# zju3dv/OnePose_Plus_Plus

Hardware: AMD Instinct MI355X
Metric: query images/sec (2D-3D match fwd) at 512x512 img x 5k pts (higher is better)
Workload: dtype f32 (operands as exact bf16 triples, f32 accumulate)

## Files before the change

onepose_plus_plus_amd/csrc/gemm_mfma.hip:

```cpp
#include <stdlib.h>

#include <mutex>
#include <type_traits>

#include <vector>

#include "opp_internal.h"

typedef float f32x16 __attribute__((ext_vector_type(16)));
typedef _Float16 f16x8 __attribute__((ext_vector_type(8)));
typedef __bf16 bf16x8 __attribute__((ext_vector_type(8)));
typedef __bf16 bf16x2 __attribute__((ext_vector_type(2)));
typedef float f32x2 __attribute__((ext_vector_type(2)));

namespace {

constexpr int lds_stride(int prec) { return prec == OPP_PREC_BF16X3 ? 52 : 36; }

__device__ __forceinline__ void opp_split4_b3(const float4 v, uint2& hi, uint2& mid, uint2& lo) {
  auto lvl = [](float a, float b, float& ra, float& rb) -> unsigned {
    const f32x2 t = {a, b};
    const unsigned p = __builtin_bit_cast(unsigned, __builtin_convertvector(t, bf16x2));
    ra = a - __uint_as_float(p << 16);
    rb = b - __uint_as_float(p & 0xffff0000u);
// ... 5 lines not shown
  const unsigned l01 = lvl(s0, s1, u0, u1), l23 = lvl(s2, s3, u2, u3);
  hi = make_uint2(h01, h23);
  mid = make_uint2(m01, m23);
  lo = make_uint2(l01, l23);
}
__device__ __forceinline__ void opp_store_split4(void* base, size_t row_bytes_off, int col, const float4 v) {
  uint2 hi, mid, lo;
  opp_split4_b3(v, hi, mid, lo);
  char* p = static_cast<char*>(base) + row_bytes_off + (col >> 3) * 48 + (col & 7) * 2;
  *reinterpret_cast<uint2*>(p) = hi;
  *reinterpret_cast<uint2*>(p + 16) = mid;
  *reinterpret_cast<uint2*>(p + 32) = lo;
}

template <int BM, int BN, int WAVES_M, int WAVES_N, bool CONV, int ABL, int DEPTH, int PREC, bool ASP>
__device__ __forceinline__ void opp_gemm_body(const OppGemm& g) {
  constexpr bool H2 = PREC == OPP_PREC_FP16X2;
  constexpr bool H3 = PREC == OPP_PREC_BF16X3;
  constexpr int kLdsStride = lds_stride(PREC);
  constexpr int NT = WAVES_M * WAVES_N * 64;
  constexpr int TM = BM / WAVES_M / 32;
  constexpr int NT32 = BN / 32;
  constexpr int TN = (NT32 + WAVES_N - 1) / WAVES_N;
  constexpr bool kRagged = (NT32 % WAVES_N) != 0;
  static_assert(!ASP || (CONV && PREC == OPP_PREC_BF16X3 && (ABL == 0 || ABL >= 200)), "pre-split activations: bf16x3 convolutions only");
  constexpr int kAblMask = ABL >= 200 ? ABL - 200 : 0;
  constexpr bool kNoGload = ABL == 91 || (kAblMask & 1), kNoLdsSt = ABL == 92 || (kAblMask & 2), kNoBar = ABL == 93 || (kAblMask & 4),
                 kNoFrag = ABL == 94 || (kAblMask & 8);
  constexpr int A_LD = ASP ? (BM * 12 + NT - 1) / NT : BM * 8 / NT;
  constexpr bool kAFrac = ASP && (BM * 12) % NT != 0;
  constexpr int kBRowsLoad = (H3 && BN == 224) ? 208 : BN;
  constexpr int B_LD = H3 ? (kBRowsLoad * 12 + NT - 1) / NT : BN * 8 / NT;
  constexpr bool kBFrac = H3 && (kBRowsLoad * 12) % NT != 0;
  constexpr bool kRing = H3 && kRagged;
  static_assert(BM % (WAVES_M * 32) == 0 && BN % 32 == 0, "tile shape");
  static_assert((BM * 8) % NT == 0 && (H3 ? (BN * 12) % NT == 0 || BN == 192 || BN == 224 : (BN * 8) % NT == 0), "load split");
  static_assert(!ASP || !((H3 && ((BN + 31) / 32 % WAVES_N) != 0)), "pre-split activations are not built for the ring tile");

  unsigned long long ts0 = 0, ts1 = 0, ts2 = 0;
  if (ABL == 9 || ABL > 90) ts0 = __builtin_readcyclecounter();
  extern __shared__ __attribute__((aligned(16))) float smem[];
  float* As = smem;
  float* Bs = smem + 2 * BM * kLdsStride;

  const int tid = threadIdx.x;
  const int lane = tid & 63;
  const int wave = tid >> 6;
  const int wm = __builtin_amdgcn_readfirstlane(kRing ? wave % WAVES_M : wave / WAVES_N);
  const int wn = __builtin_amdgcn_readfirstlane(kRing ? wave / WAVES_M : wave % WAVES_N);
  bool tile_ok[TN];
#pragma unroll
  for (int j = 0; j < TN; ++j) tile_ok[j] = kRagged ? (wn * TN + j < NT32) : true;
  const int half = lane >> 5;
  const int l31 = lane & 31;

  const int tiles_n = (g.n_store + BN - 1) / BN;
  int tile_lin = blockIdx.x;
  if (g.xcd_swizzle & 1) {
    const int nb = gridDim.x, q = nb >> 3, r = nb & 7;
    const int xcd = blockIdx.x & 7, idx = blockIdx.x >> 3;
    tile_lin = (xcd < r ? xcd * (q + 1) : r * (q + 1) + (xcd - r) * q) + idx;
  }
  const int tile_m = tile_lin / tiles_n;
  const int tile_n = tile_lin - tile_m * tiles_n;
  const int m0 = tile_m * BM;
  const int n0 = tile_n * BN;

  const int kq = tid & 7;
  const int lrow = tid >> 3;

  constexpr unsigned kOob = 0x80000000u;

  unsigned a_base0[A_LD], a_base1[A_LD], a_mask[A_LD];
  int a_lds[ASP ? A_LD : 1];
#pragma unroll
  for (int i = 0; i < A_LD; ++i) {
    const int au = tid + i * NT;
    const int arow = ASP ? au / 12 : lrow + i * (NT / 8);
    const int apiece = ASP ? au - arow * 12 : 0;
    if constexpr (ASP) a_lds[i] = arow * kLdsStride + apiece * 4;
    const int r = m0 + arow;
    if (CONV) {
      const int ox = r % g.Wout;
      const int t = r / g.Wout;
      const int oy = t % g.Hout;
      const int b = t / g.Hout;
      const int iy0 = oy * g.stride - g.pad;
      const int ix0 = ox * g.stride - g.pad;
      if constexpr (ASP) a_base0[i] = (unsigned)(((b * g.Hin + iy0) * g.Win + ix0) * g.Cin) * 6u + (unsigned)apiece * 16u;
      else a_base0[i] = (unsigned)(((b * g.Hin + iy0) * g.Win + ix0) * g.Cin + kq * 4) * 4u;
      a_base1[i] = 0;
      unsigned m = 0;
#pragma unroll
      for (int ky = 0; ky < 3; ++ky)
#pragma unroll
        for (int kx = 0; kx < 3; ++kx) {
          const bool ok = ky < g.ksize && kx < g.ksize && (unsigned)(iy0 + ky) < (unsigned)g.Hin &&
                          (unsigned)(ix0 + kx) < (unsigned)g.Win;
          m |= (ok ? 1u : 0u) << (ky * g.ksize + kx);
        }
      a_mask[i] = (r < g.M && (!kAFrac || au < BM * 12)) ? ~m : 0xffffffffu;
    } else {
      a_base0[i] = r < g.M ? (unsigned)(r * g.lda0 + kq * 4) * 4u : kOob;
      a_base1[i] = r < g.M ? (unsigned)(r * g.lda1 + kq * 4) * 4u : kOob;
      a_mask[i] = 0;
    }
  }
  constexpr bool kRingB = H3 && (NT32 % WAVES_N) != 0;
  unsigned b_base[kRingB ? 1 : B_LD];
  int b_lds[kRingB ? 1 : B_LD];
  auto ring_b = [&](int i, unsigned& base, int& lds) {
    int t = tid;
    asm volatile("" : "+v"(t));
    const int u = t + i * NT;
    const int row = u / 12, c = u - row * 12;
    const int n = n0 + row;
    base = (n < g.N && u < kBRowsLoad * 12) ? (unsigned)(n * g.ldw + c * 4) * 4u : kOob;
    lds = row * kLdsStride + c * 4;
  };
#pragma unroll
  for (int i = 0; i < (kRingB ? 0 : B_LD); ++i) {
    if (H3) {
      const int u = tid + i * NT;
      const int row = u / 12, c = u - row * 12;
      const int n = n0 + row;
      if constexpr (kBFrac) b_base[i] = (n < g.N && u < kBRowsLoad * 12) ? (unsigned)(n * g.ldw + c * 4) * 4u : kOob;
      else b_base[i] = n < g.N ? (unsigned)(n * g.ldw + c * 4) * 4u : kOob;
      b_lds[i] = row * kLdsStride + c * 4;
    } else {
      const int n = n0 + lrow + i * (NT / 8);
      b_base[i] = n < g.N ? (unsigned)(n * g.ldw + kq * 4) * 4u : kOob;
      b_lds[i] = (lrow + i * (NT / 8)) * kLdsStride + kq * 4;
    }
  }

  typedef unsigned int u32x4 __attribute__((ext_vector_type(4)));
  auto bload = [](const __amdgpu_buffer_rsrc_t r, unsigned off) -> float4 {
    const u32x4 v = __builtin_amdgcn_raw_buffer_load_b128(r, (int)off, 0, 0);
    return make_float4(__uint_as_float(v.x), __uint_as_float(v.y), __uint_as_float(v.z), __uint_as_float(v.w));
  };

  const int k_first = g.k_splits > 1 ? (int)blockIdx.y * g.k_chunks_per_split : 0;
  const int nk = g.k_splits > 1 ? max(0, min(g.k_chunks_per_split, g.K / 32 - k_first)) : g.K / 32;
  const int taps = CONV ? g.ksize * g.ksize : 1;
  const int ngrp = CONV ? g.Cin / 32 : nk;
  int cur_i = 0;
  int cur_grp = 0;
  int cur_tap = 0, cur_ky = 0, cur_kx = 0;
  int cur_k0 = k_first * 32;
  unsigned cur_past = nk > 0 ? 0u : kOob;
  unsigned eff_delta = 0, eff_sh = 31;
  int tail_i = -1;
  const int kq_lane = tid & 7;
  auto tail_lane = [&](int t, unsigned& delta, unsigned& sh) {
    const int tp = t * 8 + kq_lane;
    const int ty = tp / g.ksize, tx = tp - ty * g.ksize;
    delta = (unsigned)((ty * g.Win + tx) * g.Cin + g.tail_grp * 32 - kq_lane * 4) * 4u;
    sh = (unsigned)(31 - tp);
  };
  auto step_cursor = [&]() {
    if (CONV) {
// ... 67 lines not shown
  };
  auto load_global = [&](float4 (&a_reg)[A_LD], float4 (&b_reg)[B_LD]) {
#pragma unroll
    for (int i = 0; i < A_LD + B_LD; ++i) load_item(i, a_reg, b_reg);
  };

  auto split_h2 = [](const float4 v, uint2& hi, uint2& lo) {
    const unsigned h01 = __builtin_bit_cast(unsigned, __builtin_amdgcn_cvt_pkrtz(v.x, v.y));
    const unsigned h23 = __builtin_bit_cast(unsigned, __builtin_amdgcn_cvt_pkrtz(v.z, v.w));
    unsigned l01, l23;
    asm("v_fma_mixlo_f16 %0, %1, -1.0, %2 op_sel:[0,0,0] op_sel_hi:[1,0,0]" : "=v"(l01) : "v"(h01), "v"(v.x));
    asm("v_fma_mixhi_f16 %0, %1, -1.0, %2 op_sel:[1,0,0] op_sel_hi:[1,0,0]" : "+v"(l01) : "v"(h01), "v"(v.y));
    asm("v_fma_mixlo_f16 %0, %1, -1.0, %2 op_sel:[0,0,0] op_sel_hi:[1,0,0]" : "=v"(l23) : "v"(h23), "v"(v.z));
    asm("v_fma_mixhi_f16 %0, %1, -1.0, %2 op_sel:[1,0,0] op_sel_hi:[1,0,0]" : "+v"(l23) : "v"(h23), "v"(v.w));
    hi = make_uint2(h01, h23);
    lo = make_uint2(l01, l23);
  };
  auto split_b3 = [](const float4 v, uint2& hi, uint2& mid, uint2& lo) { opp_split4_b3(v, hi, mid, lo); };
  auto store_item = [&](int i, int buf, const float4 (&a_reg)[A_LD], const float4 (&b_reg)[B_LD]) {
    if (i < A_LD) {
      if constexpr (ASP) {
        if (!kAFrac || tid + i * NT < BM * 12) *reinterpret_cast<float4*>(As + buf * BM * kLdsStride + a_lds[i]) = a_reg[i];
        return;
      }
      float* row = As + buf * BM * kLdsStride + (lrow + i * (NT / 8)) * kLdsStride;
      if (H3) {
        uint2 hi, mid, lo;
        if (ABL == 95) {
          hi = make_uint2(__float_as_uint(a_reg[i].x), __float_as_uint(a_reg[i].y));
          mid = make_uint2(__float_as_uint(a_reg[i].z), __float_as_uint(a_reg[i].w));
          lo = hi;
        } else
        split_b3(a_reg[i], hi, mid, lo);
        float* dst = row + (kq >> 1) * 12 + (kq & 1) * 2;
        *reinterpret_cast<uint2*>(dst) = hi;
        *reinterpret_cast<uint2*>(dst + 4) = mid;
        *reinterpret_cast<uint2*>(dst + 8) = lo;
      } else if (H2) {
        uint2 hi, lo;
        split_h2(a_reg[i], hi, lo);
        float* dst = row + (kq >> 1) * 8 + (kq & 1) * 2;
        *reinterpret_cast<uint2*>(dst) = hi;
        *reinterpret_cast<uint2*>(dst + 4) = lo;
      } else {
        *reinterpret_cast<float4*>(row + kq * 4) = a_reg[i];
      }
    } else {
      if constexpr (kRingB) {
        unsigned base;
        int lds;
        ring_b(i - A_LD, base, lds);
        if (tid + (i - A_LD) * NT < kBRowsLoad * 12) *reinterpret_cast<float4*>(Bs + buf * BN * kLdsStride + lds) = b_reg[i - A_LD];
      } else if constexpr (kBFrac) {
        if (tid + (i - A_LD) * NT < kBRowsLoad * 12) *reinterpret_cast<float4*>(Bs + buf * BN * kLdsStride + b_lds[i - A_LD]) = b_reg[i - A_LD];
      } else {
        *reinterpret_cast<float4*>(Bs + buf * BN * kLdsStride + b_lds[i - A_LD]) = b_reg[i - A_LD];
      }
    }
  };
  auto store_lds = [&](int buf, const float4 (&a_reg)[A_LD], const float4 (&b_reg)[B_LD]) {
#pragma unroll
    for (int i = 0; i < A_LD + B_LD; ++i) store_item(i, buf, a_reg, b_reg);
  };

  f32x16 acc[TM][TN];
#pragma unroll
  for (int i = 0; i < TM; ++i)
// ... 13 lines not shown
    for (int i = 0; i < TM; ++i) af[i] = *reinterpret_cast<const float4*>(as + i * 32 * kLdsStride);
#pragma unroll
    for (int j = 0; j < TN; ++j)
      if (tile_ok[j]) bf[j] = *reinterpret_cast<const float4*>(bs + j * 32 * kLdsStride);
  };
  auto mfma_quarter = [&](const float4 (&af)[TM], const float4 (&bf)[TN], auto&& between) {
    int n = 0;
#pragma unroll
    for (int e = 0; e < 4; ++e) {
#pragma unroll
      for (int i = 0; i < TM; ++i) {
#pragma unroll
        for (int j = 0; j < TN; ++j) {
          if (tile_ok[j]) {
            const float av = e == 0 ? af[i].x : e == 1 ? af[i].y : e == 2 ? af[i].z : af[i].w;
            const float bv = e == 0 ? bf[j].x : e == 1 ? bf[j].y : e == 2 ? bf[j].z : bf[j].w;
            acc[i][j] = __builtin_amdgcn_mfma_f32_32x32x2f32(av, bv, acc[i][j], 0, 0, 0);
          }
          between(n);
          ++n;
        }
      }
    }
  };
  auto nothing = [](int) {};
  constexpr int kSlots = TM * TN * 4;
  constexpr int kItems = A_LD + B_LD;
  constexpr int kStride = kSlots / kItems > 0 ? kSlots / kItems : 1;

  float4 ga[DEPTH][A_LD], gb[DEPTH][B_LD];
  float4 fa[(H3 && !kRing) ? 6 : 4][TM], fb[(H3 && !kRing) ? 6 : 4][TN];
  float4 da[A_LD], db[B_LD];

  if constexpr (kRing) {
    load_global(ga[0], gb[0]);
  } else {
#pragma unroll
    for (int d = 0; d < DEPTH; ++d) {
      if (d) advance();
      load_global(ga[d], gb[d]);
    }
  }
  if constexpr (kBRowsLoad < BN) {
    for (int u = tid; u < 2 * (BN - kBRowsLoad) * kLdsStride; u += NT) {
      const int b = u / ((BN - kBRowsLoad) * kLdsStride), o = u - b * ((BN - kBRowsLoad) * kLdsStride);
      Bs[b * BN * kLdsStride + kBRowsLoad * kLdsStride + o] = 0.f;
    }
  }
  store_lds(0, ga[0], gb[0]);
  if constexpr (kRing) {
    __builtin_amdgcn_sched_barrier(0);
    advance();
    load_global(ga[1], gb[0]);
  }
  __syncthreads();
  read_frags(0, 0, fa[0], fb[0]);
  if constexpr (kRing) {
    read_frags(0, 1, fa[2], fb[2]);
    read_frags(0, 2, fa[3], fb[3]);
  } else {
    if (H2 || H3) read_frags(0, 1, fa[1], fb[1]);
    if constexpr (H3) read_frags(0, 2, fa[(H3 && !kRing) ? 2 : 0], fb[(H3 && !kRing) ? 2 : 0]);
  }

  auto chunk = [&](auto set, int lb) {
    constexpr int P = decltype(set)::value;
    constexpr int PN = (P + 1) % DEPTH;
    constexpr int A2 = ABL == 5 ? 1 : (ABL >= 6 ? 0 : ABL);
    const int B0 = A2 >= 2 ? 0 : lb;
    const int B1 = A2 >= 2 ? 0 : lb ^ 1;
    if (ABL < 1 || ABL >= 5) advance();
    if (A2 < 3) read_frags(B0, 1, fa[1], fb[1]);
    __builtin_amdgcn_sched_barrier(0);
    mfma_quarter(fa[0], fb[0], [&](int n) {
      if ((ABL < 1 || ABL >= 5) && n % kStride == 0 && n / kStride < kItems) {
        if (ABL == 5) load_item(n / kStride, da, db);
        else load_item(n / kStride, ga[P], gb[P]);
        __builtin_amdgcn_sched_barrier(0);
      }
    });
    if (ABL < 1 || ABL >= 6) {
#pragma unroll
      for (int i = kSlots / kStride; i < kItems; ++i) load_item(i, ga[P], gb[P]);
    }
    __builtin_amdgcn_sched_barrier(0);
    if (A2 < 3) read_frags(B0, 2, fa[0], fb[0]);
    __builtin_amdgcn_sched_barrier(0);
    mfma_quarter(fa[1], fb[1], nothing);
    __builtin_amdgcn_sched_barrier(0);
    if (A2 < 3) read_frags(B0, 3, fa[1], fb[1]);
// ... 207 lines not shown
    read_frags_n(B0, 5, fa[3], fb[3], tnw_c);
    __builtin_amdgcn_sched_barrier(0);
    mfma_ring(0, 2, 5, 2 * TM * TNW, tnw_c, pre);
    __builtin_amdgcn_sched_barrier(0);
    read_frags_n(B0, 4, fa[2], fb[2], tnw_c);
    __builtin_amdgcn_sched_barrier(0);
    mfma_ring(0, 5, 6, 5 * TM * TNW, tnw_c, pre);
#pragma unroll
    for (int i = kSlotsR0 / kStrideR0; i < A_LD; ++i) load_item(i, ga[P], gb[0]);
    __builtin_amdgcn_sched_barrier(0);
    mfma_ring(1, 0, 3, 0, tnw_c, [&](int n) {
      if (n % kStrideR1 == 0 && n / kStrideR1 < kItems) {
        store_item(n / kStrideR1, B1, ga[PN], gb[0]);
        __builtin_amdgcn_sched_barrier(0);
      }
    });
#pragma unroll
    for (int i = kSlotsR1 / kStrideR1; i < kItems; ++i) store_item(i, B1, ga[PN], gb[0]);
    __builtin_amdgcn_sched_barrier(0);
    __syncthreads();
    read_frags_n(B1, 0, fa[0], fb[0], tnw_c);
    read_frags_n(B1, 2, fa[3], fb[3], tnw_c);
    __builtin_amdgcn_sched_barrier(0);
    mfma_ring(1, 3, 5, 0, tnw_c, pre_b);
    __builtin_amdgcn_sched_barrier(0);
    read_frags_n(B1, 1, fa[2], fb[2], tnw_c);
    __builtin_amdgcn_sched_barrier(0);
    mfma_ring(1, 5, 6, 2 * TM * TNW, tnw_c, pre_b);
#pragma unroll
    for (int i = kSlotsR1 / kStrideRB; i < B_LD; ++i) load_item(A_LD + i, ga[P], gb[0]);
    __builtin_amdgcn_sched_barrier(0);
  };

  if (ABL == 9 || ABL > 90) ts1 = __builtin_readcyclecounter();
  if (NT == 512 && (g.xcd_swizzle & 2) && __builtin_amdgcn_readfirstlane(tid) >= 256) __builtin_amdgcn_s_setprio(1);
  if constexpr (kRing) {
    constexpr int kFull = TN, kShort = NT32 - (WAVES_N - 1) * TN;
    static_assert(DEPTH == 2 && kShort >= 1 && kShort <= TN, "ring tile");
    if (wn != WAVES_N - 1) {
      for (int c = 0; c < nk; c += 2) {
        chunk_ring(std::integral_constant<int, 0>{}, c & 1, std::integral_constant<int, kFull>{});
        chunk_ring(std::integral_constant<int, 1>{}, (c + 1) & 1, std::integral_constant<int, kFull>{});
      }
    } else {
      for (int c = 0; c < nk; c += 2) {
        chunk_ring(std::integral_constant<int, 0>{}, c & 1, std::integral_constant<int, kShort>{});
        chunk_ring(std::integral_constant<int, 1>{}, (c + 1) & 1, std::integral_constant<int, kShort>{});
      }
    }
  }
  for (int c = 0; c < (kRing ? 0 : nk); c += DEPTH) {
    if constexpr (kRing) {
    } else if constexpr (H3) {
      chunk_h3(std::integral_constant<int, 0>{}, c & 1);
      if (DEPTH > 1) chunk_h3(std::integral_constant<int, 1 % DEPTH>{}, (c + 1) & 1);
      if (DEPTH > 2) chunk_h3(std::integral_constant<int, 2 % DEPTH>{}, (c + 2) & 1);
      if (DEPTH > 3) chunk_h3(std::integral_constant<int, 3 % DEPTH>{}, (c + 3) & 1);
    } else if constexpr (H2) {
      chunk_h2(std::integral_constant<int, 0>{}, c & 1);
      if (DEPTH > 1) chunk_h2(std::integral_constant<int, 1 % DEPTH>{}, (c + 1) & 1);
      if (DEPTH > 2) chunk_h2(std::integral_constant<int, 2 % DEPTH>{}, (c + 2) & 1);
      if (DEPTH > 3) chunk_h2(std::integral_constant<int, 3 % DEPTH>{}, (c + 3) & 1);
    } else {
      chunk(std::integral_constant<int, 0>{}, c & 1);
      if (DEPTH > 1) chunk(std::integral_constant<int, 1 % DEPTH>{}, (c + 1) & 1);
      if (DEPTH > 2) chunk(std::integral_constant<int, 2 % DEPTH>{}, (c + 2) & 1);
      if (DEPTH > 3) chunk(std::integral_constant<int, 3 % DEPTH>{}, (c + 3) & 1);
    }
  }
  if (ABL == 9 || ABL > 90) ts2 = __builtin_readcyclecounter();
  if (ABL == 5) {
#pragma unroll
    for (int i = 0; i < A_LD; ++i) asm volatile("" ::"v"(da[i].x), "v"(da[i].w));
#pragma unroll
    for (int i = 0; i < B_LD; ++i) asm volatile("" ::"v"(db[i].x), "v"(db[i].w));
  }

  constexpr int kJPmax = TN < 4 ? TN : 4;
  constexpr int kOperandFloats = 2 * (BM + BN) * kLdsStride;
  constexpr int JP = (BM * (WAVES_N * kJPmax * 32 + 4) <= kOperandFloats) ? kJPmax
                     : (BM * (WAVES_N * 2 * 32 + 4) <= kOperandFloats && kJPmax >= 2) ? 2 : 1;
  constexpr int NPASS = (TN + JP - 1) / JP;
  constexpr int WP = WAVES_N * JP * 32;
  constexpr int CS = WP + 4;
  static_assert((size_t)BM * CS * 4 <= (size_t)2 * (BM + BN) * kLdsStride * 4, "C tile must fit the operand LDS");
  float* Cs = smem;
  const bool scale_on = (g.out_mul != 1.f) || (g.out_div != 1.f);
  const bool vec_ok = g.vec_epilogue != 0;
  const float h2_inv = (H2 && g.h2_inv != nullptr) ? *g.h2_inv : 1.f;
  if (H2 || scale_on) {
#pragma unroll
    for (int i = 0; i < TM; ++i)
#pragma unroll
      for (int j = 0; j < TN; ++j)
#pragma unroll
        for (int r = 0; r < 16; ++r) {
          const float cv0 = H2 ? acc[i][j][r] * h2_inv : acc[i][j][r];
          acc[i][j][r] = scale_on ? (cv0 * g.out_mul) / g.out_div : cv0;
        }
  }
  if (g.col_mask != nullptr) {
#pragma unroll
    for (int j = 0; j < TN; ++j) {
      const int col = n0 + wn * TN * 32 + j * 32 + l31;
      const float add = (col < g.n_store && g.col_mask[col] == 0.f) ? -1e9f : 0.f;
#pragma unroll
      for (int i = 0; i < TM; ++i)
#pragma unroll
        for (int r = 0; r < 16; ++r) acc[i][j][r] += add;
    }
  }
  if constexpr (H2) {
    if (g.nonfinite != nullptr) {
      bool bad = false;
#pragma unroll
      for (int i = 0; i < TM; ++i)
#pragma unroll
        for (int j = 0; j < TN; ++j)
#pragma unroll
          for (int r = 0; r < 16; ++r) bad |= !(fabsf(acc[i][j][r]) <= 3.4028235e38f);
      if (__builtin_amdgcn_ballot_w64(bad) != 0ull && lane == 0) atomicOr(g.nonfinite, 1);
    }
  }
#pragma unroll
  for (int ps = 0; ps < NPASS; ++ps) {
    __syncthreads();
#pragma unroll
    for (int i = 0; i < TM; ++i)
#pragma unroll
      for (int jj = 0; jj < JP; ++jj) {
        const int j = ps * JP + jj;
        if (j < TN && tile_ok[j]) {
#pragma unroll
          for (int r = 0; r < 16; ++r) {
            const int lr = wm * TM * 32 + i * 32 + (r & 3) + 8 * (r >> 2) + 4 * half;
            Cs[lr * CS + wn * JP * 32 + jj * 32 + l31] = acc[i][j][r];
          }
        }
      }
    __syncthreads();
    if constexpr (NPASS == 1 && !kRagged && (NT % BM) == 0 && kOperandFloats - BM * CS >= 2 * (NT / BM) * BM + 2 * WAVES_M * WP) {
      if (g.stat_rowmax != nullptr) {
        constexpr int kParts = NT / BM;
        constexpr int kQ = WP / 4 / kParts;
        float* sc_r = Cs + BM * CS;
        float* sc_c = sc_r + 2 * kParts * BM;
        const int ncols = min(WP, g.n_store - n0);
        const int nrows = min(BM, g.M - m0);
        {
          const int lr = tid % BM, part = tid / BM;
          const float* rowp = Cs + lr * CS + part * kQ * 4;
          float mx = -INFINITY;
#pragma unroll 4
          for (int q = 0; q < kQ; ++q) {
            const float4 v = *reinterpret_cast<const float4*>(rowp + q * 4);
            const int c = (part * kQ + q) * 4;
            mx = fmaxf(mx, c + 0 < ncols ? v.x : -INFINITY);
            mx = fmaxf(mx, c + 1 < ncols ? v.y : -INFINITY);
            mx = fmaxf(mx, c + 2 < ncols ? v.z : -INFINITY);
            mx = fmaxf(mx, c + 3 < ncols ? v.w : -INFINITY);
          }
          sc_r[part * BM + lr] = mx;
          __syncthreads();
          mx = sc_r[lr];
#pragma unroll
          for (int pp = 1; pp < kParts; ++pp) mx = fmaxf(mx, sc_r[pp * BM + lr]);
          float sm = 0.f;
#pragma unroll 4
          for (int q = 0; q < kQ; ++q) {
            const float4 v = *reinterpret_cast<const float4*>(rowp + q * 4);
            const int c = (part * kQ + q) * 4;
            sm += c + 0 < ncols ? __expf(v.x - mx) : 0.f;
            sm += c + 1 < ncols ? __expf(v.y - mx) : 0.f;
            sm += c + 2 < ncols ? __expf(v.z - mx) : 0.f;
// ... 31 lines not shown
            float m = sc_c[wn * TN * 32 + j * 32 + l31];
#pragma unroll
            for (int w = 1; w < WAVES_M; ++w) m = fmaxf(m, sc_c[w * WP + wn * TN * 32 + j * 32 + l31]);
            cmx[j] = m;
          }
          __syncthreads();
#pragma unroll
          for (int j = 0; j < TN; ++j) {
            float sm = 0.f;
#pragma unroll
            for (int i = 0; i < TM; ++i)
#pragma unroll
              for (int r = 0; r < 16; ++r) sm += rvalid(i, r) ? __expf(sval(i, j, r) - cmx[j]) : 0.f;
            sm += __shfl_xor(sm, 32, 64);
            if (half == 0) sc_c[wm * WP + wn * TN * 32 + j * 32 + l31] = sm;
          }
          __syncthreads();
          if (wm == 0 && half == 0) {
#pragma unroll
            for (int j = 0; j < TN; ++j) {
              const int c = wn * TN * 32 + j * 32 + l31;
              if (c < ncols) {
                float tot = sc_c[c];
#pragma unroll
                for (int w = 1; w < WAVES_M; ++w) tot += sc_c[w * WP + c];
                g.stat_colmax[(size_t)tile_m * g.n_store + n0 + c] = cmx[j];
                g.stat_colsum[(size_t)tile_m * g.n_store + n0 + c] = tot;
              }
            }
          }
        }
      }
    }
    if constexpr (NPASS == 1 && !kRagged && (WP == 256 || WP == 128)) {
      if (g.ln_gamma != nullptr) {
        constexpr int VPT = WP / 64, NW = WAVES_M * WAVES_N, RPW = 4;
        typedef float vec_t __attribute__((ext_vector_type(VPT)));
        static_assert(BM % (NW * RPW) == 0 || BM / NW < RPW, "rows per wave");
        const vec_t gmv = *reinterpret_cast<const vec_t*>(g.ln_gamma + lane * VPT);
        const vec_t btv = *reinterpret_cast<const vec_t*>(g.ln_beta + lane * VPT);
        constexpr int ROWS_W = BM / NW;
        constexpr int GRP = ROWS_W < RPW ? ROWS_W : RPW;
#pragma unroll
        for (int r0 = 0; r0 < ROWS_W; r0 += GRP) {
          float v[GRP][VPT], rv[GRP][VPT], sm[GRP], mean[GRP], rstd[GRP];
#pragma unroll
          for (int r = 0; r < GRP; ++r) {
            const int lr = wave * ROWS_W + r0 + r;
            const vec_t t = *reinterpret_cast<const vec_t*>(Cs + lr * CS + lane * VPT);
            const bool ok = m0 + lr < g.M;
            vec_t rt;
#pragma unroll
            for (int i = 0; i < VPT; ++i) rt[i] = 0.f;
            if (ok && g.ln_res) rt = *reinterpret_cast<const vec_t*>(g.ln_res + (size_t)(m0 + lr) * g.ln_ldres + lane * VPT);
            sm[r] = 0.f;
#pragma unroll
            for (int i = 0; i < VPT; ++i) {
              v[r][i] = t[i];
              rv[r][i] = rt[i];
              sm[r] += t[i];
            }
          }
#pragma unroll
          for (int r = 0; r < GRP; ++r) sm[r] = opp_wave_sum_dpp(sm[r]);
#pragma unroll
          for (int r = 0; r < GRP; ++r) {
            mean[r] = sm[r] / (float)WP;
// ... 2 lines not shown
            for (int i = 0; i < VPT; ++i) {
              const float d = v[r][i] - mean[r];
              sm[r] = opp_ln_sq_acc(d, sm[r]);
            }
          }
#pragma unroll
          for (int r = 0; r < GRP; ++r) sm[r] = opp_wave_sum_dpp(sm[r]);
#pragma unroll
          for (int r = 0; r < GRP; ++r) rstd[r] = 1.0f / sqrtf(sm[r] / (float)WP + g.ln_eps);
#pragma unroll
          for (int r = 0; r < GRP; ++r) {
            const int lr = wave * ROWS_W + r0 + r;
            if (m0 + lr < g.M) {
              vec_t o;
#pragma unroll
              for (int i = 0; i < VPT; ++i) {
                float y = opp_ln_affine(v[r][i], mean[r], rstd[r], gmv[i], btv[i]);
                if (g.ln_res) y = rv[r][i] + y;
                o[i] = y;
              }
              *reinterpret_cast<vec_t*>(g.C + (size_t)(m0 + lr) * g.ldc + lane * VPT) = o;
            }
          }
        }
        continue;
      }
    }
    for (int u = tid; u < BM * (WP / 4); u += NT) {
      const int lr = u / (WP / 4);
      const int lc = (u - lr * (WP / 4)) * 4;
      const int wn2 = lc / (JP * 32);
      const int j = ps * JP + (lc - wn2 * JP * 32) / 32;
      const int row = m0 + lr;
      const int col = n0 + wn2 * TN * 32 + j * 32 + (lc & 31);
      if (j >= TN || (kRagged && wn2 * TN + j >= NT32) || row >= g.M || col >= g.n_store) continue;
      const float4 cv = *reinterpret_cast<const float4*>(Cs + lr * CS + lc);
      float v[4] = {cv.x, cv.y, cv.z, cv.w};
      const int nval = g.n_store - col < 4 ? g.n_store - col : 4;
      if (g.bias) {
        if (vec_ok) {
          const float4 bv = *reinterpret_cast<const float4*>(g.bias + col);
          v[0] += bv.x; v[1] += bv.y; v[2] += bv.z; v[3] += bv.w;
        } else {
          for (int e = 0; e < nval; ++e) v[e] += g.bias[col + e];
        }
      }
      if (g.res_mode == OPP_RES_DIRECT) {
        const float* rp = g.R + (size_t)row * g.ldr + col;
        if (vec_ok) {
          const float4 rv = *reinterpret_cast<const float4*>(rp);
          v[0] += rv.x; v[1] += rv.y; v[2] += rv.z; v[3] += rv.w;
        } else {
          for (int e = 0; e < nval; ++e) v[e] += rp[e];
        }
      } else if (g.res_mode == OPP_RES_BILINEAR2X) {
#pragma clang fp contract(off)
        const int ox = row % g.Wout;
        const int t = row / g.Wout;
        const int oy = t % g.Hout;
        const int b = t / g.Hout;
        const float sy = g.res_sy * (float)oy;
        const float sx = g.res_sx * (float)ox;
        int y0 = (int)sy;
        if (y0 > g.Hr - 1) y0 = g.Hr - 1;
        int x0 = (int)sx;
        if (x0 > g.Wr - 1) x0 = g.Wr - 1;
        const int y1 = y0 + (y0 < g.Hr - 1 ? 1 : 0);
        const int x1 = x0 + (x0 < g.Wr - 1 ? 1 : 0);
// ... 118 lines not shown
    }
    if (out != nullptr) out[i] = make_float4(v[0], v[1], v[2], v[3]);
  }
}

template <typename K>
void set_lds_once(K k, size_t lds, OppLdsOnce& once) {
  opp_lds_opt_in(reinterpret_cast<const void*>(k), lds, once);
}

template <int BM, int BN, int WAVES_M, int WAVES_N, int DEPTH, int PREC>
int launch_prec(const OppGemm& g, hipStream_t stream, size_t extra_lds) {
  constexpr int NT = WAVES_M * WAVES_N * 64;
  constexpr bool kNarrowB3 = BM == 128 && (BN == 192 || BN == 224) && NT == 512 && PREC == OPP_PREC_BF16X3;
  constexpr bool ok = (PREC == OPP_PREC_FP32 && BN != 192 && BN != 224) ||
                      (DEPTH == 2 && (NT == 512 || (BM == 64 && BN == 64) || (PREC == OPP_PREC_FP16X2 && BM == 128 && BN == 128)) &&
                       (BN == 128 || BN == 64 || BN == 256 || kNarrowB3) &&
                       (PREC != OPP_PREC_BF16X3 || (BN * 12) % NT == 0 || kNarrowB3) && (PREC != OPP_PREC_BF16X3 || BM * BN / NT <= 64 || kNarrowB3));
  if constexpr (ok) {
    const size_t lds = (size_t)2 * (BM + BN) * lds_stride(PREC) * sizeof(float) + extra_lds;
    const int tiles = opp_cdiv(g.M, BM) * opp_cdiv(g.n_store, BN);
    constexpr bool kAspBuilt = PREC == OPP_PREC_BF16X3 && DEPTH == 2 && !kNarrowB3 && (NT == 512 || (BM == 64 && BN == 64));
    if (g.conv && g.a_split) {
      if constexpr (kAspBuilt) {
        auto k = opp_gemm_asp_kernel<BM, BN, WAVES_M, WAVES_N, 0, DEPTH, PREC>;
        static OppLdsOnce attr_done;
        set_lds_once(k, lds, attr_done);
        hipLaunchKernelGGL(k, dim3(tiles, g.k_splits > 1 ? g.k_splits : 1), dim3(NT), lds, stream, g);
      } else {
        opp_set_error("gemm: tile %dx%d is not built for pre-split activations", BM, BN);
        return OPP_ERR_UNSUPPORTED;
      }
    } else if (g.conv) {
      auto k = opp_gemm_kernel<BM, BN, WAVES_M, WAVES_N, true, 0, DEPTH, PREC>;
      static OppLdsOnce attr_done;
      set_lds_once(k, lds, attr_done);
      hipLaunchKernelGGL(k, dim3(tiles, g.k_splits > 1 ? g.k_splits : 1), dim3(NT), lds, stream, g);
    } else {
      auto k = opp_gemm_kernel<BM, BN, WAVES_M, WAVES_N, false, 0, DEPTH, PREC>;
      static OppLdsOnce attr_done;
      set_lds_once(k, lds, attr_done);
      hipLaunchKernelGGL(k, dim3(tiles, g.k_splits > 1 ? g.k_splits : 1), dim3(NT), lds, stream, g);
    }
    OPP_CHECK_LAUNCH("opp_gemm_kernel");
    return OPP_OK;
  } else {
    opp_set_error("gemm: tile %dx%d on %d waves is not built for operand precision %d", BM, BN, WAVES_M * WAVES_N, PREC);
    return OPP_ERR_UNSUPPORTED;
  }
}

template <int BM, int BN, int WAVES_M, int WAVES_N, int DEPTH = 2>
int launch_cfg(const OppGemm& g, hipStream_t stream) {
#ifdef OPP_TUNING
  static const size_t extra_lds = getenv("OPP_EXTRA_LDS") ? (size_t)atoi(getenv("OPP_EXTRA_LDS")) : 0;
#else
  constexpr size_t extra_lds = 0;
#endif
  switch (g.prec) {
    case OPP_PREC_FP32: return launch_prec<BM, BN, WAVES_M, WAVES_N, DEPTH, OPP_PREC_FP32>(g, stream, extra_lds);
#ifdef OPP_TUNING
    case OPP_PREC_FP16X2: return launch_prec<BM, BN, WAVES_M, WAVES_N, DEPTH, OPP_PREC_FP16X2>(g, stream, extra_lds);
#else
    case OPP_PREC_FP16X2: opp_set_error("gemm: fp16x2 operands are built into the tuning library only"); return OPP_ERR_UNSUPPORTED;
#endif
    case OPP_PREC_BF16X3: return launch_prec<BM, BN, WAVES_M, WAVES_N, DEPTH, OPP_PREC_BF16X3>(g, stream, extra_lds);
    default: opp_set_error("gemm: unknown operand precision %d", g.prec); return OPP_ERR_INVALID;
  }
}

// ... 219 lines not shown
      OPP_CHECK_LAUNCH("splitk_epilogue_kernel");
      return OPP_OK;
    }
  }
  const bool auto_cfg = cfg < 0;
  if (cfg < 0) cfg = choose_tile(g);
  OPP_CHECK_ARG(g.stat_rowmax == nullptr || (g.prec == OPP_PREC_BF16X3 ? (cfg == 25 || cfg == 20) : cfg == 0),
                "gemm: fused softmax statistics need the 128x128 tile (config 0; bf16x3: config 25, or 20 = 256x128)");
  if (g.ln_gamma != nullptr) {
    if (auto_cfg || (cfg != 30 && cfg != 26)) cfg = g.n_store == 256 ? 30 : 26;
    auto al = [](const void* p) { return (reinterpret_cast<uintptr_t>(p) & 15) == 0; };
    OPP_CHECK_ARG(g.ln_beta && ((cfg == 30 && g.n_store == 256) || (cfg == 26 && g.n_store == 128)) && g.N == g.n_store && !g.bias &&
                      g.act == OPP_ACT_NONE && g.res_mode == OPP_RES_NONE && g.ldc % 4 == 0 && al(g.C) && al(g.ln_gamma) &&
                      al(g.ln_beta) && (!g.ln_res || (al(g.ln_res) && g.ln_ldres % 4 == 0)),
                  "gemm: fused LayerNorm needs a 256- or 128-column output, no bias/activation/residual mode, aligned operands");
  }
  OppProfScope prof_scope(g.conv && g.k_splits > 1 ? (int)OPP_PROF_CONV_SPLITK : opp_prof_gemm_symbol(cfg, g.conv ? 1 : (g.stat_rowmax ? 2 : 0)), stream,
                          g.alg_flops > 0.0 ? g.alg_flops : 2.0 * (double)g.M * (double)g.N * (double)g.K);
  int rc;
  switch (cfg) {
    case 0: rc = launch_cfg<128, 128, 2, 2>(g, stream); break;
    case 1: rc = launch_cfg<64, 128, 2, 2>(g, stream); break;
    case 2: rc = launch_cfg<64, 64, 2, 2>(g, stream); break;
    case 10: rc = launch_cfg<128, 128, 2, 2, 3>(g, stream); break;
    case 11: rc = launch_cfg<128, 128, 2, 2, 4>(g, stream); break;
    case 20: rc = launch_cfg<256, 128, 4, 2>(g, stream); break;
    case 22: rc = launch_cfg<128, 256, 2, 4>(g, stream); break;
    case 24: rc = launch_cfg<128, 192, 4, 2>(g, stream); break;
    case 25: rc = launch_cfg<128, 128, 4, 2>(g, stream); break;
    case 27:
      if (g.prec != OPP_PREC_BF16X3 || g.n_store > 224 || (g.n_real > 208 && g.n_real != g.n_store)) {
        opp_set_error("gemm: tile config 27 (128 x 224) is a bf16x3 tile for outputs of <= 208 real and <= 224 stored columns");
        rc = OPP_ERR_UNSUPPORTED;
      } else {
        rc = launch_cfg<128, 224, 4, 2>(g, stream);
      }
      break;
    case 26: rc = launch_cfg<64, 128, 2, 4>(g, stream); break;
    case 30: rc = launch_cfg<64, 256, 2, 4>(g, stream); break;
    default:
#ifdef OPP_TUNING
      rc = launch_tuning_cfg(g, cfg, stream);
#else
      opp_set_error("gemm: unknown tile config %d", cfg);
      rc = OPP_ERR_INVALID;
#endif
      break;
  }
  return rc;
}

extern "C" int opp_debug_timestamps(void* buf) {
#ifdef OPP_TUNING
  g_dbg_ts = static_cast<unsigned long long*>(buf);
  opp_gemm_ss_debug_timestamps(buf, getenv("OPP_SS_TS_MODE") ? atoi(getenv("OPP_SS_TS_MODE")) : 0);
  return OPP_OK;
#else
  (void)buf;
  opp_set_error("opp_debug_timestamps: library built without -DOPP_TUNING");
  return OPP_ERR_UNSUPPORTED;
#endif
}

int opp_gemm_launch(const OppGemm& g, hipStream_t stream) { return opp_gemm_launch_cfg(g, -1, stream); }

int opp_gemm_choose_tile(const OppGemm& g) {
// ... 5 lines not shown
```

Measured before the change: 527.5.

## Use 16x16x32 MFMA main loop with swizzled LDS for bf16x3 convolutions

Adds a separate main loop for bf16x3 implicit-GEMM convolutions that uses 16x16x32 bf16 MFMA instructions instead of the 32x32 path. Global loads and LDS stores are interleaved across quadrant halves. LDS piece offsets gain an XOR swizzle to reduce bank conflicts, and the accumulator and epilogue layouts change to match. Convolutions that would have used config 27 (128x224) are routed to a 128x256 tile instead. The cost is a more complex schedule, and the C-tile fused epilogues (col_mask, rowmax, layernorm) are disabled on this path.

Measured after the change: 560.7 (median of 6 runs). 6.3% higher.

```diff
diff --git a/onepose_plus_plus_amd/csrc/gemm_mfma.hip b/onepose_plus_plus_amd/csrc/gemm_mfma.hip
--- a/onepose_plus_plus_amd/csrc/gemm_mfma.hip
+++ b/onepose_plus_plus_amd/csrc/gemm_mfma.hip
@@ -61,7 +61,12 @@
   constexpr int kBRowsLoad = (H3 && BN == 224) ? 208 : BN;
   constexpr int B_LD = H3 ? (kBRowsLoad * 12 + NT - 1) / NT : BN * 8 / NT;
   constexpr bool kBFrac = H3 && (kBRowsLoad * 12) % NT != 0;
-  constexpr bool kRing = H3 && kRagged;
+  constexpr bool kRing = H3 && kRagged && !CONV;
+  constexpr bool kM16 = H3 && CONV;
+  constexpr int NB16 = kM16 ? kBRowsLoad / 16 : 1;
+  constexpr int NBW = kM16 ? (NB16 + WAVES_N - 1) / WAVES_N : 1;
+  constexpr int MB = 2 * TM;
+  static_assert(!kM16 || (kBRowsLoad % 16 == 0 && (!kRagged || WAVES_N == 2)), "16 x 16 tile shape");
   static_assert(BM % (WAVES_M * 32) == 0 && BN % 32 == 0, "tile shape");
   static_assert((BM * 8) % NT == 0 && (H3 ? (BN * 12) % NT == 0 || BN == 192 || BN == 224 : (BN * 8) % NT == 0), "load split");
   static_assert(!ASP || !((H3 && ((BN + 31) / 32 % WAVES_N) != 0)), "pre-split activations are not built for the ring tile");
@@ -75,8 +80,8 @@
   const int tid = threadIdx.x;
   const int lane = tid & 63;
   const int wave = tid >> 6;
-  const int wm = __builtin_amdgcn_readfirstlane(kRing ? wave % WAVES_M : wave / WAVES_N);
-  const int wn = __builtin_amdgcn_readfirstlane(kRing ? wave / WAVES_M : wave % WAVES_N);
+  const int wm = __builtin_amdgcn_readfirstlane((H3 && kRagged) ? wave % WAVES_M : wave / WAVES_N);
+  const int wn = __builtin_amdgcn_readfirstlane((H3 && kRagged) ? wave / WAVES_M : wave % WAVES_N);
   bool tile_ok[TN];
 #pragma unroll
   for (int j = 0; j < TN; ++j) tile_ok[j] = kRagged ? (wn * TN + j < NT32) : true;
@@ -99,6 +104,8 @@
   const int lrow = tid >> 3;
 
   constexpr unsigned kOob = 0x80000000u;
+  auto kswz = [](int r) -> int { return kM16 ? ((r >> 2) ^ (r >> 3)) & 1 : 0; };
+  auto piece_off = [&](int r, int c) -> int { return r * kLdsStride + (((c / 3) ^ kswz(r)) * 3 + c % 3) * 4; };
 
   unsigned a_base0[A_LD], a_base1[A_LD], a_mask[A_LD];
   int a_lds[ASP ? A_LD : 1];
@@ -107,7 +114,7 @@
     const int au = tid + i * NT;
     const int arow = ASP ? au / 12 : lrow + i * (NT / 8);
     const int apiece = ASP ? au - arow * 12 : 0;
-    if constexpr (ASP) a_lds[i] = arow * kLdsStride + apiece * 4;
+    if constexpr (ASP) a_lds[i] = piece_off(arow, apiece);
     const int r = m0 + arow;
     if (CONV) {
       const int ox = r % g.Wout;
@@ -155,7 +162,7 @@
       const int n = n0 + row;
       if constexpr (kBFrac) b_base[i] = (n < g.N && u < kBRowsLoad * 12) ? (unsigned)(n * g.ldw + c * 4) * 4u : kOob;
       else b_base[i] = n < g.N ? (unsigned)(n * g.ldw + c * 4) * 4u : kOob;
-      b_lds[i] = row * kLdsStride + c * 4;
+      b_lds[i] = piece_off(row, c);
     } else {
       const int n = n0 + lrow + i * (NT / 8);
       b_base[i] = n < g.N ? (unsigned)(n * g.ldw + kq * 4) * 4u : kOob;
@@ -289,7 +296,7 @@
           lo = hi;
         } else
         split_b3(a_reg[i], hi, mid, lo);
-        float* dst = row + (kq >> 1) * 12 + (kq & 1) * 2;
+        float* dst = row + ((kq >> 1) ^ kswz(lrow + i * (NT / 8))) * 12 + (kq & 1) * 2;
         *reinterpret_cast<uint2*>(dst) = hi;
         *reinterpret_cast<uint2*>(dst + 4) = mid;
         *reinterpret_cast<uint2*>(dst + 8) = lo;
@@ -369,7 +376,7 @@
   float4 fa[(H3 && !kRing) ? 6 : 4][TM], fb[(H3 && !kRing) ? 6 : 4][TN];
   float4 da[A_LD], db[B_LD];
 
-  if constexpr (kRing) {
+  if constexpr (kRing || kM16) {
     load_global(ga[0], gb[0]);
   } else {
 #pragma unroll
@@ -378,7 +385,7 @@
       load_global(ga[d], gb[d]);
     }
   }
-  if constexpr (kBRowsLoad < BN) {
+  if constexpr (kBRowsLoad < BN && !kM16) {
     for (int u = tid; u < 2 * (BN - kBRowsLoad) * kLdsStride; u += NT) {
       const int b = u / ((BN - kBRowsLoad) * kLdsStride), o = u - b * ((BN - kBRowsLoad) * kLdsStride);
       Bs[b * BN * kLdsStride + kBRowsLoad * kLdsStride + o] = 0.f;
@@ -389,10 +396,15 @@
     __builtin_amdgcn_sched_barrier(0);
     advance();
     load_global(ga[1], gb[0]);
+  } else if constexpr (kM16) {
+    __builtin_amdgcn_sched_barrier(0);
+    advance();
+    load_global(ga[0], gb[0]);
   }
   __syncthreads();
-  read_frags(0, 0, fa[0], fb[0]);
-  if constexpr (kRing) {
+  if constexpr (!kM16) read_frags(0, 0, fa[0], fb[0]);
+  if constexpr (kM16) {
+  } else if constexpr (kRing) {
     read_frags(0, 1, fa[2], fb[2]);
     read_frags(0, 2, fa[3], fb[3]);
   } else {
@@ -666,6 +678,118 @@
     __builtin_amdgcn_sched_barrier(0);
   };
 
+
+  typedef float f32x4 __attribute__((ext_vector_type(4)));
+  constexpr int NBH0 = (NBW + 1) / 2;
+  f32x4 acc4[kM16 ? MB : 1][kM16 ? NBW : 1];
+  float4 fa4[3][kM16 ? MB : 1], fb4[3][kM16 ? NBW : 1];
+  if constexpr (kM16) {
+#pragma unroll
+    for (int i = 0; i < MB; ++i)
+#pragma unroll
+      for (int j = 0; j < NBW; ++j) acc4[i][j] = f32x4{0.f, 0.f, 0.f, 0.f};
+  }
+  const int f16off = (lane & 15) * kLdsStride + (((lane >> 4) ^ kswz(lane & 15)) * 3) * 4;
+  const int a_frag16 = wm * TM * 32 * kLdsStride + f16off;
+  const int b_frag16 = wn * NBW * 16 * kLdsStride + f16off;
+  auto read_a16 = [&](int buf, auto h_c) {
+    constexpr int H = decltype(h_c)::value;
+    const float* as = As + buf * BM * kLdsStride + a_frag16;
+#pragma unroll
+    for (int i = H * TM; i < H * TM + TM; ++i)
+#pragma unroll
+      for (int p = 0; p < 3; ++p) fa4[p][i] = *reinterpret_cast<const float4*>(as + i * 16 * kLdsStride + p * 4);
+  };
+  auto read_b16 = [&](int buf, auto v_c, auto nbw_c) {
+    constexpr int V = decltype(v_c)::value, NBL = decltype(nbw_c)::value;
+    constexpr int j0 = V ? NBH0 : 0, j1 = V ? NBL : (NBH0 < NBL ? NBH0 : NBL);
+    const float* bs = Bs + buf * BN * kLdsStride + b_frag16;
+#pragma unroll
+    for (int j = j0; j < j1; ++j)
+#pragma unroll
+      for (int p = 0; p < 3; ++p) fb4[p][j] = *reinterpret_cast<const float4*>(bs + j * 16 * kLdsStride + p * 4);
+  };
+  auto quad16 = [&](auto h_c, auto v_c, auto nbw_c, auto&& between) {
+    constexpr int H = decltype(h_c)::value, V = decltype(v_c)::value, NBL = decltype(nbw_c)::value;
+    constexpr int j0 = V ? NBH0 : 0, j1 = V ? NBL : (NBH0 < NBL ? NBH0 : NBL);
+    constexpr int PA[6] = {2, 0, 1, 1, 0, 0};
+    constexpr int PB[6] = {0, 2, 1, 0, 1, 0};
+    int n = 0;
+#pragma unroll
+    for (int pr = 0; pr < 6; ++pr)
+#pragma unroll
+      for (int i = H * TM; i < H * TM + TM; ++i)
+#pragma unroll
+        for (int j = j0; j < j1; ++j) {
+          acc4[i][j] = __builtin_amdgcn_mfma_f32_16x16x32_bf16(as_b8(fa4[PA[pr]][i]), as_b8(fb4[PB[pr]][j]), acc4[i][j], 0, 0, 0);
+          between(n);
+          ++n;
+        }
+  };
+  auto chunk_m16 = [&](auto set, int lb, auto nbw_c) {
+    constexpr int P = decltype(set)::value;
+    constexpr int NBL = decltype(nbw_c)::value;
+    constexpr int O = P & 1;
+    constexpr int kSl0 = 6 * TM * (O ? NBL - NBH0 : (NBH0 < NBL ? NBH0 : NBL));
+    constexpr int kSl1 = 6 * TM * (O ? (NBH0 < NBL ? NBH0 : NBL) : NBL - NBH0);
+    constexpr int kSt0 = kSl0 / kItems > 0 ? kSl0 / kItems : 1;
+    constexpr int kSt1 = kSl1 / kItems > 0 ? kSl1 / kItems : 1;
+    using I0 = std::integral_constant<int, 0>;
+    using I1 = std::integral_constant<int, 1>;
+    const int B0 = lb, B1 = lb ^ 1;
+    advance();
+    if (!kNoFrag) {
+      if constexpr (O == 0) read_b16(B0, I1{}, nbw_c);
+      else read_b16(B0, I0{}, nbw_c);
+      read_a16(B0, I1{});
+    }
+    __builtin_amdgcn_sched_barrier(0);
+    auto hand = [&](int n) {
+      if (n % kSt0 == 0 && n / kSt0 < kItems) {
+        if (!kNoLdsSt) store_item(n / kSt0, B1, ga[0], gb[0]);
+        __builtin_amdgcn_sched_barrier(0);
+      }
+    };
+    auto pre = [&](int n) {
+      if (n % kSt1 == 0 && n / kSt1 < kItems) {
+        if (!kNoGload) load_item(n / kSt1, ga[0], gb[0]);
+        __builtin_amdgcn_sched_barrier(0);
+      }
+    };
+    if constexpr (O == 0) quad16(I0{}, I0{}, nbw_c, hand);
+    else quad16(I0{}, I1{}, nbw_c, hand);
+#pragma unroll
+    for (int i = kSl0 / kSt0; i < kItems; ++i)
+      if (!kNoLdsSt) store_item(i, B1, ga[0], gb[0]);
+    __builtin_amdgcn_sched_barrier(0);
+    if constexpr (O == 0) quad16(I0{}, I1{}, nbw_c, pre);
+    else quad16(I0{}, I0{}, nbw_c, pre);
+#pragma unroll
+    for (int i = kSl1 / kSt1; i < kItems; ++i)
+      if (!kNoGload) load_item(i, ga[0], gb[0]);
+    __builtin_amdgcn_sched_barrier(0);
+    if (!kNoBar) __syncthreads();
+    if (!kNoFrag) read_a16(B1, I0{});
+    __builtin_amdgcn_sched_barrier(0);
+    if constexpr (O == 0) quad16(I1{}, I1{}, nbw_c, nothing);
+    else quad16(I1{}, I0{}, nbw_c, nothing);
+    __builtin_amdgcn_sched_barrier(0);
+    if (!kNoFrag) {
+      if constexpr (O == 0) read_b16(B1, I1{}, nbw_c);
+      else read_b16(B1, I0{}, nbw_c);
+    }
+    __builtin_amdgcn_sched_barrier(0);
+    if constexpr (O == 0) quad16(I1{}, I0{}, nbw_c, nothing);
+    else quad16(I1{}, I1{}, nbw_c, nothing);
+    __builtin_amdgcn_sched_barrier(0);
+  };
+  if constexpr (kM16) {
+    if (!kNoFrag) {
+      read_a16(0, std::integral_constant<int, 0>{});
+      read_b16(0, std::integral_constant<int, 0>{}, std::integral_constant<int, NBW>{});
+    }
+  }
+
   if (ABL == 9 || ABL > 90) ts1 = __builtin_readcyclecounter();
   if (NT == 512 && (g.xcd_swizzle & 2) && __builtin_amdgcn_readfirstlane(tid) >= 256) __builtin_amdgcn_s_setprio(1);
   if constexpr (kRing) {
@@ -683,8 +807,23 @@
       }
     }
   }
-  for (int c = 0; c < (kRing ? 0 : nk); c += DEPTH) {
-    if constexpr (kRing) {
+  if constexpr (kM16) {
+    static_assert(DEPTH == 2, "16 x 16 loop: the two quadrant orders alternate over a chunk pair");
+    constexpr int kShort16 = NB16 - (WAVES_N - 1) * NBW;
+    if (!kRagged || wn != WAVES_N - 1) {
+      for (int c = 0; c < nk; c += 2) {
+        chunk_m16(std::integral_constant<int, 0>{}, c & 1, std::integral_constant<int, NBW>{});
+        chunk_m16(std::integral_constant<int, 1>{}, (c + 1) & 1, std::integral_constant<int, NBW>{});
+      }
+    } else {
+      for (int c = 0; c < nk; c += 2) {
+        chunk_m16(std::integral_constant<int, 0>{}, c & 1, std::integral_constant<int, kShort16>{});
+        chunk_m16(std::integral_constant<int, 1>{}, (c + 1) & 1, std::integral_constant<int, kShort16>{});
+      }
+    }
+  }
+  for (int c = 0; c < ((kRing || kM16) ? 0 : nk); c += DEPTH) {
+    if constexpr (kRing || kM16) {
     } else if constexpr (H3) {
       chunk_h3(std::integral_constant<int, 0>{}, c & 1);
       if (DEPTH > 1) chunk_h3(std::integral_constant<int, 1 % DEPTH>{}, (c + 1) & 1);
@@ -714,15 +853,24 @@
   constexpr int kOperandFloats = 2 * (BM + BN) * kLdsStride;
   constexpr int JP = (BM * (WAVES_N * kJPmax * 32 + 4) <= kOperandFloats) ? kJPmax
                      : (BM * (WAVES_N * 2 * 32 + 4) <= kOperandFloats && kJPmax >= 2) ? 2 : 1;
-  constexpr int NPASS = (TN + JP - 1) / JP;
-  constexpr int WP = WAVES_N * JP * 32;
+  constexpr int NPASS = kM16 ? 1 : (TN + JP - 1) / JP;
+  constexpr int WP = kM16 ? BN : WAVES_N * JP * 32;
   constexpr int CS = WP + 4;
   static_assert((size_t)BM * CS * 4 <= (size_t)2 * (BM + BN) * kLdsStride * 4, "C tile must fit the operand LDS");
   float* Cs = smem;
   const bool scale_on = (g.out_mul != 1.f) || (g.out_div != 1.f);
   const bool vec_ok = g.vec_epilogue != 0;
   const float h2_inv = (H2 && g.h2_inv != nullptr) ? *g.h2_inv : 1.f;
-  if (H2 || scale_on) {
+  if constexpr (kM16) {
+    if (scale_on) {
+#pragma unroll
+      for (int i = 0; i < MB; ++i)
+#pragma unroll
+        for (int j = 0; j < NBW; ++j)
+#pragma unroll
+          for (int r = 0; r < 4; ++r) acc4[i][j][r] = (acc4[i][j][r] * g.out_mul) / g.out_div;
+    }
+  } else if (H2 || scale_on) {
 #pragma unroll
     for (int i = 0; i < TM; ++i)
 #pragma unroll
@@ -733,7 +881,7 @@
           acc[i][j][r] = scale_on ? (cv0 * g.out_mul) / g.out_div : cv0;
         }
   }
-  if (g.col_mask != nullptr) {
+  if (!kM16 && g.col_mask != nullptr) {
 #pragma unroll
     for (int j = 0; j < TN; ++j) {
       const int col = n0 + wn * TN * 32 + j * 32 + l31;
@@ -759,6 +907,15 @@
 #pragma unroll
   for (int ps = 0; ps < NPASS; ++ps) {
     __syncthreads();
+    if constexpr (kM16) {
+#pragma unroll
+      for (int i = 0; i < MB; ++i)
+#pragma unroll
+        for (int j = 0; j < NBW; ++j)
+#pragma unroll
+          for (int r = 0; r < 4; ++r)
+            Cs[(wm * TM * 32 + i * 16 + (lane >> 4) * 4 + r) * CS + wn * NBW * 16 + j * 16 + (lane & 15)] = acc4[i][j][r];
+    } else
 #pragma unroll
     for (int i = 0; i < TM; ++i)
 #pragma unroll
@@ -773,7 +930,7 @@
         }
       }
     __syncthreads();
-    if constexpr (NPASS == 1 && !kRagged && (NT % BM) == 0 && kOperandFloats - BM * CS >= 2 * (NT / BM) * BM + 2 * WAVES_M * WP) {
+    if constexpr (!kM16 && NPASS == 1 && !kRagged && (NT % BM) == 0 && kOperandFloats - BM * CS >= 2 * (NT / BM) * BM + 2 * WAVES_M * WP) {
       if (g.stat_rowmax != nullptr) {
         constexpr int kParts = NT / BM;
         constexpr int kQ = WP / 4 / kParts;
@@ -871,7 +1028,7 @@
         }
       }
     }
-    if constexpr (NPASS == 1 && !kRagged && (WP == 256 || WP == 128)) {
+    if constexpr (!kM16 && NPASS == 1 && !kRagged && (WP == 256 || WP == 128)) {
       if (g.ln_gamma != nullptr) {
         constexpr int VPT = WP / 64, NW = WAVES_M * WAVES_N, RPW = 4;
         typedef float vec_t __attribute__((ext_vector_type(VPT)));
@@ -940,8 +1097,8 @@
       const int wn2 = lc / (JP * 32);
       const int j = ps * JP + (lc - wn2 * JP * 32) / 32;
       const int row = m0 + lr;
-      const int col = n0 + wn2 * TN * 32 + j * 32 + (lc & 31);
-      if (j >= TN || (kRagged && wn2 * TN + j >= NT32) || row >= g.M || col >= g.n_store) continue;
+      const int col = kM16 ? n0 + lc : n0 + wn2 * TN * 32 + j * 32 + (lc & 31);
+      if ((!kM16 && (j >= TN || (kRagged && wn2 * TN + j >= NT32))) || row >= g.M || col >= g.n_store) continue;
       const float4 cv = *reinterpret_cast<const float4*>(Cs + lr * CS + lc);
       float v[4] = {cv.x, cv.y, cv.z, cv.w};
       const int nval = g.n_store - col < 4 ? g.n_store - col : 4;
@@ -1126,10 +1283,15 @@
         return OPP_ERR_UNSUPPORTED;
       }
     } else if (g.conv) {
-      auto k = opp_gemm_kernel<BM, BN, WAVES_M, WAVES_N, true, 0, DEPTH, PREC>;
-      static OppLdsOnce attr_done;
-      set_lds_once(k, lds, attr_done);
-      hipLaunchKernelGGL(k, dim3(tiles, g.k_splits > 1 ? g.k_splits : 1), dim3(NT), lds, stream, g);
+      if constexpr (PREC == OPP_PREC_BF16X3 && BN == 224) {
+        opp_set_error("gemm: bf16x3 convolutions have no 224-column tile (config 27 runs them on 128 x 256)");
+        return OPP_ERR_UNSUPPORTED;
+      } else {
+        auto k = opp_gemm_kernel<BM, BN, WAVES_M, WAVES_N, true, 0, DEPTH, PREC>;
+        static OppLdsOnce attr_done;
+        set_lds_once(k, lds, attr_done);
+        hipLaunchKernelGGL(k, dim3(tiles, g.k_splits > 1 ? g.k_splits : 1), dim3(NT), lds, stream, g);
+      }
     } else {
       auto k = opp_gemm_kernel<BM, BN, WAVES_M, WAVES_N, false, 0, DEPTH, PREC>;
       static OppLdsOnce attr_done;
@@ -1415,6 +1577,8 @@
       if (g.prec != OPP_PREC_BF16X3 || g.n_store > 224 || (g.n_real > 208 && g.n_real != g.n_store)) {
         opp_set_error("gemm: tile config 27 (128 x 224) is a bf16x3 tile for outputs of <= 208 real and <= 224 stored columns");
         rc = OPP_ERR_UNSUPPORTED;
+      } else if (g.conv && g.prec == OPP_PREC_BF16X3) {
+        rc = launch_cfg<128, 256, 2, 4>(g, stream);
       } else {
         rc = launch_cfg<128, 224, 4, 2>(g, stream);
       }
```
